# wzx99/DCFP

Measured on AMD Instinct MI355X. Metric: training images/sec at 1024x2048 DeepLabv3-R101, higher is better.
Workload: dtype f32; 1 GPU; DeepLabv3-resnet101+ASPP os8, 4x3x1024x2048 per GPU, CE+0.4*deepsup CE (fused upsample), 3x3 stride-1 convs with >= 256 channels as fp32 Winograd F(2x2,3x3) (fwd / dgrad / wgrad), all other convs direct implicit GEMM, EIC step, SGD m0.9 wd5e-4; global_batch=4, parallelism=dp1

## Files before the change

dcfp_amd/_lib.py:

```python
import ctypes as C
import os
import subprocess
import threading

_HERE = os.path.dirname(os.path.abspath(__file__))
LIB_PATH = os.environ.get("DCFP_LIB") or os.path.join(_HERE, "libdcfp_hip.so")
CSRC = os.path.join(_HERE, "csrc")

_lib = None
_lock = threading.Lock()


class ConvDesc(C.Structure):
    _fields_ = [(n, C.c_int32) for n in
                ("N", "Cin", "H", "W", "Cout", "KH", "KW", "stride", "pad", "dil", "Hout", "Wout",
                 "x_pitch", "dy_pitch")]


class ConvF16Desc(C.Structure):
    _fields_ = [(n, C.c_int32) for n in
                ("N", "H", "W", "Cin8", "x_pitch", "Cout", "K", "stride", "pad", "dil", "Hout", "Wout",
                 "y_pitch", "y_off", "res_pitch", "res_off", "relu")]


# ... 54 lines not shown

AUG_SATURATION, AUG_HUE = 1, 2
SGD_CHUNK = 16384
CONV_FWD, CONV_DGRAD, CONV_WGRAD = 0, 1, 2
E_BADDESC, E_UNSUPPORTED, E_WORKSPACE = -1, -2, -3

_P, _I, _L, _F, _Z = C.c_void_p, C.c_int, C.c_int64, C.c_float, C.c_size_t
_D = C.POINTER(ConvDesc)
_R = C.POINTER(BnRunning)
_H = C.POINTER(ConvF16Desc)
_H8 = C.POINTER(ConvF8Desc)

SIGNATURES = {
    "dcfp_abi_version": (_I, []),
    "dcfp_conv2d_workspace_bytes": (_Z, [_D, _I]),
    "dcfp_conv2d_wp_layout": (_I, [_D, _I, C.POINTER(WpEntry)]),
    "dcfp_conv2d_permute_weights_multi_f32": (_I, [_P, _I, _L, _P]),
    "dcfp_conv2d_pitch_supported": (_I, [_D]),
    "dcfp_conv2d_kernel_name": (_I, [_D, _I, C.c_char_p, _I]),
    "dcfp_conv2d_executed_fraction": (C.c_double, [_D, _I]),
    "dcfp_conv2d_workspace_is_scratch": (_I, [_D, _I]),
    "dcfp_conv2d_dgrad_fanin_supported": (_I, [_D]),
    "dcfp_conv2d_dgrad_fanin_f32_nchw": (_I, [_D, _P, _L, _P, _P, _P, _P, _P, _Z, _I, _P]),
    "dcfp_conv2d_dgrad_fanin_red_slots": (_L, [_D]),
    "dcfp_conv2d_dgrad_fanin_red_f32_nchw": (_I, [_D, _P, _L, _P, _P, _P, _P, _P, _P, _P, _P, _P, _Z, _I, _P]),
    "dcfp_bn_bwd_sums_from_partials_f32": (_I, [_P, _L, _I, _P, _F, _P, _P, _P, _P, _P]),
    "dcfp_conv2d_xform_bytes": (_Z, [_D]),
    "dcfp_conv2d_fwd_keep_f32_nchw": (_I, [_D, _P, _P, _P, _L, _P, _Z, _P, _P, _Z, _P]),
    "dcfp_conv2d_wgrad_kept_f32_nchw": (_I, [_D, _P, _L, _P, _Z, _P, _P, _Z, _P]),
    "dcfp_conv2d_fwd_f32_nchw": (_I, [_D, _P, _P, _P, _P, _L, _P, _Z, _I, _P]),
    "dcfp_conv2d_fwd_fused_f32_nchw": (_I, [_D, _P, _P, _P, _P, _P, _I, _P, _P, _Z, _I, _P]),
    "dcfp_conv2d_dgrad_f32_nchw": (_I, [_D, _P, _L, _P, _P, _I, _P, _Z, _I, _P]),
    "dcfp_conv2d_wgrad_f32_nchw": (_I, [_D, _P, _L, _P, _P, _P, _P, _Z, _P]),
    "dcfp_bn_workspace_bytes": (_Z, [_I, _I, _I]),
    "dcfp_bn_stats_f32": (_I, [_P, _L, _I, _I, _I, _P, _P, _R, _P, _Z, _P]),
    "dcfp_bn_apply_f32": (_I, [_P, _P, _P, _P, _P, _F, _P, _I, _P, _L, _I, _I, _I, _I, _I, _P]),
    "dcfp_bn_bwd_reduce_f32": (_I, [_P, _L, _P, _P, _L, _P, _P, _P, _P, _F, _I, _I, _I, _I, _P, _P, _P, _P,
                                    _P, _Z, _P]),
    "dcfp_bn_update_running_f32": (_I, [_P, _P, _I, _F, _F, _P, _P, _P, _P]),
    "dcfp_syncbn_combine_f32": (_I, [_P, _I, _I, _P, _P, _P, _R, _P]),
    "dcfp_syncbn_p2p_mailbox_bytes": (_Z, [_I, _I]),
    "dcfp_p2p_alloc": (_I, [_Z, _I, C.POINTER(C.c_void_p)]),
    "dcfp_p2p_free": (_I, [_P]),
    "dcfp_p2p_export": (_I, [_P, _P]),
    "dcfp_p2p_import": (_I, [_P, C.POINTER(C.c_void_p)]),
    "dcfp_p2p_unmap": (_I, [_P]),
    "dcfp_syncbn_p2p_exchange_f32": (_I, [C.POINTER(C.c_void_p), _I, _I, C.c_uint32, _I, _P, _I, _I, _P, _R,
                                          C.c_uint32, _P, _P]),
    "dcfp_bn_apply_relu_mask_f32": (_I, [_P, _P, _P, _P, _P, _F, _P, _P, _P, _I, _I, _I, _P]),
    "dcfp_conv2d_fwd_stat_slots": (_L, [_D, _P, _L]),
    "dcfp_conv2d_fwd_stats_f32_nchw": (_I, [_D, _P, _P, _P, _L, _P, _P, _Z, _I, _P]),
    "dcfp_bn_stats_from_partials_f32": (_I, [_P, _L, _I, _I, _P, _P, _R, _P]),
    "dcfp_bn_bwd_apply_f32": (_I, [_P, _L, _P, _P, _L, _P, _P, _P, _P, _F, _P, _P, _F, _P, _I, _P, _P,
                                   _I, _I, _I, _I, _I, _P]),
    "dcfp_bn_bwd_fused_sync_bytes": (_Z, [_I, _I, _I]),
    "dcfp_bn_bwd_fused_f32": (_I, [_P, _L, _P, _P, _L, _P, _P, _P, _P, _F, _F, _I, _P, _P, _I, _I, _I, _I, _I,
                                   _P, _P, _P, _P, _P, _Z, C.c_uint32, C.c_uint32, _P, _P]),
    "dcfp_maxpool3x3s2_fwd_f32": (_I, [_P, _P, _P, _I, _I, _I, _I, _I, _I, _P]),
    "dcfp_maxpool3x3s2_bwd_f32": (_I, [_P, _P, _P, _I, _I, _I, _I, _I, _I, _P]),
    "dcfp_rowsum_f32": (_I, [_P, _L, _P, _F, _I, _I, _I, _P]),
    "dcfp_broadcast_hw_f32": (_I, [_P, _F, _P, _L, _I, _I, _I, _I, _P]),
    "dcfp_add_f32": (_I, [_P, _P, _P, _L, _P]),
    "dcfp_channel_scale_f32": (_I, [_P, _P, _P, _I, _I, _I, _P]),
    "dcfp_upsample_bilinear_fwd_f32": (_I, [_P, _P, _I, _I, _I, _I, _I, _I, _I, _P]),
    "dcfp_upsample_bilinear_bwd_f32": (_I, [_P, _P, _I, _I, _I, _I, _I, _I, _I, _P]),
    "dcfp_resize_bilinear_into_f32": (_I, [_P, _L, _I, _I, _I, _I, _P, _L, _I, _I, _I, _I, _P]),
# ... 94 lines not shown
```

dcfp_amd/csrc/conv_igemm2.hip:

```cpp
#include "igemm2_common.h"
#include <queue>
#include <vector>
#include <stdio.h>
#include <stdlib.h>

namespace {

__device__ __forceinline__ int wp_row(int m, int perm8) {
    if (!perm8) return m;
    const int j = m & 255;
    return (m & ~255) + 32 * (j & 7) + (j >> 3);
}

__global__ void __launch_bounds__(256)
permute_weights_kernel(const float* __restrict__ w, float* __restrict__ wp, int T, int Ck, int CkP,
                       int M, int Mpad, int sAm, int sAc, int perm8) {
    const long long total = (long long)T * CkP * Mpad;
    for (long long i = (long long)blockIdx.x * 256 + threadIdx.x; i < total;
         i += (long long)gridDim.x * 256) {
        const int m = wp_row((int)(i % Mpad), perm8);
        const long long r = i / Mpad;
        const int c = (int)(r % CkP);
        const int t = (int)(r / CkP);
        float v = 0.f;
        if (m < M && c < Ck) v = w[(long long)m * sAm + (long long)c * sAc + t];
        wp[i] = v;
    }
}

constexpr int kWpBlockElems = DCFP_WP_BLOCK_ELEMS;
__global__ void __launch_bounds__(256)
permute_weights_multi_kernel(const DcfpWpEntry* __restrict__ table, int n) {
    const long long blk = blockIdx.x;
    int lo = 0, hi = n - 1;
    while (lo < hi) {
        const int mid = (lo + hi + 1) >> 1;
        if (table[mid].first_block <= blk) lo = mid; else hi = mid - 1;
    }
    const DcfpWpEntry e = table[lo];
    const long long base = (blk - e.first_block) * kWpBlockElems;
    if (e.perm8 >= 2) {
        const long long pairs = (long long)e.CkP * e.Mpad;
#pragma unroll 1
        for (int u = 0; u < kWpBlockElems / 256; ++u) {
            const long long i = base + u * 256 + threadIdx.x;
            if (i >= pairs) return;
            wino_filter2_pair(e.w, e.sAm, e.sAc, e.perm8 == 3, e.M, e.Ck, e.Mpad, i, e.wp);
        }
        return;
    }
    const long long total = (long long)e.T * e.CkP * e.Mpad;
#pragma unroll
    for (int u = 0; u < kWpBlockElems / 256; ++u) {
        const long long i = base + u * 256 + threadIdx.x;
        if (i >= total) return;
        const int m = wp_row((int)(i % e.Mpad), e.perm8);
        const long long r = i / e.Mpad;
        const int c = (int)(r % e.CkP);
        const int t = (int)(r / e.CkP);
        float v = 0.f;
        if (m < e.M && c < e.Ck) v = e.w[(long long)m * e.sAm + (long long)c * e.sAc + t];
        e.wp[i] = v;
    }
}

__device__ __forceinline__ float half_xor(float v, int mask) {
    switch (mask) {
        case 1: return __builtin_bit_cast(float, __builtin_amdgcn_ds_swizzle(__builtin_bit_cast(int, v), (1 << 10) | 0x1f));
        case 2: return __builtin_bit_cast(float, __builtin_amdgcn_ds_swizzle(__builtin_bit_cast(int, v), (2 << 10) | 0x1f));
        case 4: return __builtin_bit_cast(float, __builtin_amdgcn_ds_swizzle(__builtin_bit_cast(int, v), (4 << 10) | 0x1f));
        case 8: return __builtin_bit_cast(float, __builtin_amdgcn_ds_swizzle(__builtin_bit_cast(int, v), (8 << 10) | 0x1f));
        default: return __builtin_bit_cast(float, __builtin_amdgcn_ds_swizzle(__builtin_bit_cast(int, v), (16 << 10) | 0x1f));
    }
}

template <int TAPS, int TM, int TN, int WM, int WN, bool SD, bool ACC, int KB = 16>
__global__ void __launch_bounds__(64 * WM * WN, (TM * TN <= 8 && WM * WN == 4 && !ACC) ? 2 : 1)
igemm2_kernel(const Igemm2Params p) {
    constexpr int BK = KB;
    constexpr int NPART = BK / 4;
    constexpr int BM = WM * TM * 32, BN = WN * TN * 32, NT = 64 * WM * WN;
    constexpr int AX = BM / 4;
    constexpr int AROWS = (NT / AX) < BK ? (NT / AX) : BK;
// ... 1047 lines not shown
```

dcfp_amd/csrc/conv_wgrad.hip:

```cpp
#include "common.h"
#include <stdio.h>
#include <stdlib.h>
#include <string.h>
#include <type_traits>

int dcfp_wgrad3_launch(const float* dy, long long dy_nstride, const float* x, long long x_nstride,
                       float* out, int N, int M, int Cin, int T, int H, int W, int Ho, int Wo, int pad,
                       int dil, int Kpix, int kchunk, int splits, int tiles_m, int tiles_n,
                       hipStream_t stream);

namespace {

typedef float f32x16 __attribute__((ext_vector_type(16)));

constexpr int BK = 16;
constexpr int BKP = 20;

struct WgradParams {
    const float* dy;
    const float* x;
    float* out;
    long long dy_nstride, x_nstride;
    int N, M, Cin, Nn;
    int H, W, Ho, Wo, P, stride, pad, dil;
// ... 890 lines not shown
    const Plan pl = make_plan(d);
    const char* args = pl.cfg == 0 ? "4,4,2,2" : pl.cfg == 1 ? "2,4,2,2" : pl.cfg == 3 ? "4,2,2,2" :
                       pl.cfg == 4 ? "4,1,2,2" : pl.cfg == 5 ? "2,3,2,2" : "2,2,1,1";
    if (wgrad3_ok(d, pl.cfg)) return snprintf(buf, buf_len, "wgrad3_kernel<%d>", d->KH * d->KW);
    if (pl.wide) return snprintf(buf, buf_len, "wgrad_dma_kernel<%d,false,true>", d->KH * d->KW);
    if (wgrad_dma_ok(d, pl.cfg))
        return snprintf(buf, buf_len, "wgrad_dma_kernel<%d,%s>", d->KH * d->KW,
                        (wgrad_dma_mixed(d) && !(d->x_pitch && d->x_pitch != d->W)) ? "true" : "false");
    return snprintf(buf, buf_len, "wgrad2_kernel<%d,%s>", d->KH * d->KW, args);
}

bool dcfp_wino_wgrad_ok(int N, int H, int W, int d, int M, int C);
size_t dcfp_wino_wgrad_workspace_bytes(int N, int H, int W, int d, int M, int C);
double dcfp_wino_exec_fraction(int N, int H, int W, int d, int M, int Ck);
int dcfp_wino_wgrad_run(const float* dy, long long dy_nstride, int dy_pitch, const float* x, long long x_nstride,
                        int x_pitch, float* dw, int N, int M, int C, int H, int W, int d, void* workspace,
                        size_t workspace_bytes, hipStream_t stream, const float* xform_in = nullptr);
extern "C" size_t dcfp_conv2d_xform_bytes(const DcfpConvDesc* d);

static double wino_wgrad_fused_rate() {
    static const double v = [] { const char* e = getenv("DCFP_WINO_WGRAD_RATE"); return (e ? atof(e) : 118.0) * 1e12; }();
    return v;
}
static bool wino_wgrad_fused_forced() {
    static const bool v = [] { const char* e = getenv("DCFP_WINO_WGRAD_FUSED"); return e && atoi(e) == 2; }();
    return v;
}

bool dcfp_wino_wgrad_fused_ok(int N, int H, int W, int d, int M, int C, long long x_nstride, int x_pitch,
                              long long dy_nstride, int dy_pitch);
size_t dcfp_wino_wgrad_fused_workspace_bytes(int N, int H, int W, int d, int M, int C);
int dcfp_wino_wgrad_fused_run(const float* dy, long long dy_nstride, int dy_pitch, const float* x, long long x_nstride,
                              int x_pitch, float* dw, int N, int M, int C, int H, int W, int d, void* workspace,
                              size_t workspace_bytes, hipStream_t stream);

static int wino_wgrad_kind(const DcfpConvDesc* d) {
    static const int mode = [] { const char* e = getenv("DCFP_CONV_WINOGRAD"); return e ? atoi(e) : 1; }();
    if (mode == 0) return 0;
    if (d->KH != 3 || d->KW != 3 || d->stride != 1 || d->pad != d->dil || d->Hout != d->H || d->Wout != d->W) return 0;
    if (math_bf16x3()) return 0;
    const int xp = d->x_pitch ? d->x_pitch : d->W, dyp = d->dy_pitch ? d->dy_pitch : d->Wout;
    const bool batched = dcfp_wino_wgrad_ok(d->N, d->H, d->W, d->dil, d->Cout, d->Cin);
    const bool fused = dcfp_wino_wgrad_fused_ok(d->N, d->H, d->W, d->dil, d->Cout, d->Cin, (long long)d->Cin * d->H * xp, xp,
                                                (long long)d->Cout * d->Hout * dyp, dyp);
    if (!batched && !fused) return 0;
    if (mode == 2) return fused ? 2 : 1;
    const double pix = (double)d->N * d->H * d->W;
    const double nominal = 2.0 * pix * d->Cout * (double)d->Cin * 9.0;
    const bool dense_d1 = wgrad_dma_mixed(d) && !(d->x_pitch && d->x_pitch != d->W);
    const bool ragged = d->Cout % 256 != 0 || (d->Cin * 9) % 256 != 0;
    const double dpad = ragged ? (double)((d->Cout + 31) / 32 * 32) / d->Cout * (double)((d->Cin * 9 + 255) / 256 * 256) / (d->Cin * 9) * 1.15
                               : 1.0;
    const double t_direct = nominal * dpad / (d->Cout < 128 ? 100e12 : dense_d1 ? 123e12 : 130e12);
    const double f = dcfp_wino_exec_fraction(d->N, d->H, d->W, d->dil, d->Cout, d->Cin);
    double t_b = 1e30, t_f = 1e30;
    if (batched) {
        const double tiles = f * 9.0 / 16.0 * pix;
        const double pad2 = (double)((d->Cout + 255) / 256 * 256) / d->Cout * (double)((d->Cin + 255) / 256 * 256) / d->Cin;
        t_b = nominal * f * pad2 / 125e12 + (4.0 * pix * d->Cin + 64.0 * tiles * d->Cin) / 4.2e12 +
              (4.0 * pix * d->Cout + 64.0 * tiles * d->Cout) / 5.0e12 + 30e-6;
    }
    if (fused) {
        const double pad64 = (double)((d->Cout + 63) / 64 * 64) / d->Cout * (double)((d->Cin + 63) / 64 * 64) / d->Cin;
        t_f = nominal * f * pad64 / wino_wgrad_fused_rate() + 40e-6;
    }
    if (fused && (t_f <= t_b || wino_wgrad_fused_forced())) return t_f < 0.97 * t_direct ? 2 : 0;
    return t_b < 0.97 * t_direct ? 1 : 0;
}
static bool wino_wgrad_pass(const DcfpConvDesc* d) { return wino_wgrad_kind(d) != 0; }

bool dcfp_wgrad_is_winograd(const DcfpConvDesc* d) { return wino_wgrad_pass(d); }
bool dcfp_wgrad_wants_xform(const DcfpConvDesc* d) { return wino_wgrad_kind(d) == 1; }

double dcfp_wgrad_exec_fraction(const DcfpConvDesc* d) {
    return wino_wgrad_pass(d) ? dcfp_wino_exec_fraction(d->N, d->H, d->W, d->dil, d->Cout, d->Cin) : 1.0;
}

size_t dcfp_conv2d_fwd_dgrad_workspace_bytes_(const DcfpConvDesc* d, int pass);

extern "C" size_t dcfp_conv2d_workspace_bytes(const DcfpConvDesc* d, int pass) {
    if (pass == DCFP_CONV_FWD || pass == DCFP_CONV_DGRAD) return dcfp_conv2d_fwd_dgrad_workspace_bytes_(d, pass);
    if (pass != DCFP_CONV_WGRAD || check_desc(d) != DCFP_OK) return 0;
    if (dcfp_stem_shape(d)) return dcfp_stem_wgrad_workspace_bytes(d);
    if (const int wk = wino_wgrad_kind(d)) {
        const size_t b1 = dcfp_wino_wgrad_ok(d->N, d->H, d->W, d->dil, d->Cout, d->Cin)
                              ? dcfp_wino_wgrad_workspace_bytes(d->N, d->H, d->W, d->dil, d->Cout, d->Cin) : 0;
        if (wk == 1) return b1;
        const size_t b2 = dcfp_wino_wgrad_fused_workspace_bytes(d->N, d->H, d->W, d->dil, d->Cout, d->Cin);
        const Plan pl = make_plan(d);
        const size_t b0 = pl.splits > 1 ? (size_t)pl.splits * d->Cout * d->Cin * d->KH * d->KW * sizeof(float) : 0;
        const size_t m = b1 > b0 ? b1 : b0;
        return b2 > m ? b2 : m;
    }
    const Plan pl = make_plan(d);
    if (pl.splits <= 1) return 0;
    return (size_t)pl.splits * d->Cout * d->Cin * d->KH * d->KW * sizeof(float);
}

extern "C" int dcfp_conv2d_wgrad_f32_nchw(const DcfpConvDesc* d, const float* dy,
                                          int64_t dy_nstride, const float* x, float* dw, float* db,
                                          void* workspace, size_t workspace_bytes,
                                          dcfp_stream_t stream) {
    int rc = check_desc(d);
    if (rc) return rc;
    if (!dy || !x || !dw) return DCFP_E_BADDESC;
    if (dcfp_gemv_shape(d) && !db)
        return dcfp_gemv_wgrad(d, dy, dy_nstride, x, dw, dcfp_s(stream));
    if (dcfp_stem_shape(d) && !db)
        return dcfp_stem_wgrad(d, dy, dy_nstride, x, dw, workspace, workspace_bytes, dcfp_s(stream));
    int wk = wino_wgrad_kind(d);
    if (wk == 2) {
        const int dyp = d->dy_pitch ? d->dy_pitch : d->Wout, xp = d->x_pitch ? d->x_pitch : d->W;
        const long long dyn = dy_nstride ? dy_nstride : (long long)d->Cout * d->Hout * dyp;
        if (!dcfp_wino_wgrad_fused_ok(d->N, d->H, d->W, d->dil, d->Cout, d->Cin, (long long)d->Cin * d->H * xp, xp, dyn, dyp))
            wk = dcfp_wino_wgrad_ok(d->N, d->H, d->W, d->dil, d->Cout, d->Cin) ? 1 : 0;
    }
    if (wk) {
        const int dyp = d->dy_pitch ? d->dy_pitch : d->Wout, xp = d->x_pitch ? d->x_pitch : d->W;
        const long long dyn = dy_nstride ? dy_nstride : (long long)d->Cout * d->Hout * dyp;
        if (db && dyp != d->Wout) return DCFP_E_UNSUPPORTED;
        if (wk == 2) {
            rc = dcfp_wino_wgrad_fused_run(dy, dyn, dyp, x, (long long)d->Cin * d->H * xp, xp, dw, d->N, d->Cout, d->Cin, d->H,
                                           d->W, d->dil, workspace, workspace_bytes, dcfp_s(stream));
        } else
            rc = dcfp_wino_wgrad_run(dy, dyn, dyp, x, (long long)d->Cin * d->H * xp, xp, dw, d->N, d->Cout, d->Cin, d->H, d->W,
                                     d->dil, workspace, workspace_bytes, dcfp_s(stream));
        if (rc) return rc;
        if (db)
            hipLaunchKernelGGL(bias_grad_kernel, dim3((unsigned)d->Cout), dim3(1024), 0, dcfp_s(stream), dy, dyn, db, d->N,
                               d->Hout * d->Wout, (int)((d->Hout * d->Wout) % 4 == 0 && dyn % 4 == 0 && dcfp_aligned16(dy)));
        DCFP_RETURN_LAUNCH();
    }
    const Plan pl = make_plan(d);
    const int T = d->KH * d->KW;
    const long long wn = (long long)d->Cout * d->Cin * T;
    const size_t need = pl.splits > 1 ? (size_t)pl.splits * wn * sizeof(float) : 0;
    if (need && (!workspace || workspace_bytes < need)) return DCFP_E_WORKSPACE;
    WgradParams p;
    p.dy = dy; p.x = x;
    p.out = pl.splits > 1 ? static_cast<float*>(workspace) : dw;
    p.x_pitch = d->x_pitch ? d->x_pitch : d->W;
    p.dy_pitch = d->dy_pitch ? d->dy_pitch : d->Wout;
    const bool pitched = p.x_pitch != d->W || p.dy_pitch != d->Wout;
    if (pitched && !dcfp_wgrad_pitch_ok(d)) return DCFP_E_UNSUPPORTED;
    if (db && p.dy_pitch != d->Wout) return DCFP_E_UNSUPPORTED;
    p.dy_nstride = dy_nstride ? dy_nstride : (long long)d->Cout * d->Hout * p.dy_pitch;
    p.x_nstride = (long long)d->Cin * d->H * p.x_pitch;
    p.N = d->N; p.M = d->Cout; p.Cin = d->Cin; p.Nn = d->Cin * T;
    p.H = d->H; p.W = d->W; p.Ho = d->Hout; p.Wo = d->Wout; p.P = d->Hout * d->Wout;
    p.stride = d->stride; p.pad = d->pad; p.dil = d->dil;
    if ((long long)d->N * p.P >= (1LL << 30)) return DCFP_E_UNSUPPORTED;
    p.Kpix = d->N * p.P;
    p.kchunk = pl.kchunk; p.splits = pl.splits; p.tiles_m = pl.tiles_m; p.tiles_n = pl.tiles_n;
    p.quad_ok = (d->Wout % 4 == 0) ? 1 : 0;
    p.batch = 1; p.dy_bstride = p.x_bstride = 0;
    {
// ... 8 lines not shown
    else if (pl.wide) {
        const long long blocks = (long long)pl.tiles_m * pl.tiles_n * pl.splits;
        if (blocks > 0x7fffffffLL) return DCFP_E_UNSUPPORTED;
        rc = T == 1 ? launch_dma<1, false, true>(p, blocks, dcfp_s(stream)) : launch_dma<9, false, true>(p, blocks, dcfp_s(stream));
    } else if (wgrad_dma_ok(d, pl.cfg)) {
        const long long blocks = (long long)pl.tiles_m * pl.tiles_n * pl.splits;
        if (blocks > 0x7fffffffLL) return DCFP_E_UNSUPPORTED;
        rc = T == 1 ? (pl.half ? launch_dma<1, false, false, false, true>(p, blocks, dcfp_s(stream)) : launch_dma<1, false>(p, blocks, dcfp_s(stream)))
                    : (wgrad_dma_mixed(d) && p.x_pitch == d->W) ? launch_dma<9, true>(p, blocks, dcfp_s(stream))
                                                                 : launch_dma<9, false>(p, blocks, dcfp_s(stream));
    } else
        rc = T == 1 ? launch_taps<1>(p, pl, dcfp_s(stream)) : launch_taps<9>(p, pl, dcfp_s(stream));
    if (rc) return rc;
    if (pl.splits > 1) {
        if (wn % 4 == 0 && dcfp_aligned16(workspace) && dcfp_aligned16(dw)) {
            const long long n4 = wn / 4;
            hipLaunchKernelGGL(splitk_reduce_vec4_kernel, dim3((unsigned)((n4 + 255) / 256)), dim3(256), 0,
                               dcfp_s(stream), static_cast<const float*>(workspace), dw, n4, wn, pl.splits);
        } else {
            long long b = (wn + 255) / 256;
            if (b > 4096) b = 4096;
            hipLaunchKernelGGL(splitk_reduce_kernel, dim3((unsigned)b), dim3(256), 0, dcfp_s(stream),
                               static_cast<const float*>(workspace), dw, wn, pl.splits);
        }
    }
    if (db) {
        hipLaunchKernelGGL(bias_grad_kernel, dim3((unsigned)d->Cout), dim3(1024), 0, dcfp_s(stream),
                           dy, p.dy_nstride, db, d->N, p.P,
                           (int)(p.P % 4 == 0 && p.dy_nstride % 4 == 0 && dcfp_aligned16(dy) && p.dy_pitch == d->Wout));
    }
    DCFP_RETURN_LAUNCH();
}

extern "C" int dcfp_conv2d_wgrad_kept_f32_nchw(const DcfpConvDesc* d, const float* dy, int64_t dy_nstride,
                                               const float* xform, size_t xform_bytes, float* dw, void* workspace,
                                               size_t workspace_bytes, dcfp_stream_t stream) {
    int rc = check_desc(d);
    if (rc) return rc;
    if (!dy || !xform || !dw) return DCFP_E_BADDESC;
    const size_t need = dcfp_conv2d_xform_bytes(d);
    if (need == 0) return DCFP_E_UNSUPPORTED;
    if (xform_bytes < need || !dcfp_aligned16(xform)) return DCFP_E_WORKSPACE;
    const int dyp = d->dy_pitch ? d->dy_pitch : d->Wout;
    const long long dyn = dy_nstride ? dy_nstride : (long long)d->Cout * d->Hout * dyp;
    return dcfp_wino_wgrad_run(dy, dyn, dyp, nullptr, 0, 0, dw, d->N, d->Cout, d->Cin, d->H, d->W, d->dil, workspace,
                               workspace_bytes, dcfp_s(stream), xform);
}
```

dcfp_amd/csrc/conv_winograd3.hip:

```cpp
#include "wino_patch.h"
#include <stdlib.h>

namespace {

constexpr int GBK = 8;
constexpr int GKH = 144;
constexpr int GHALF = 2 * GKH;
constexpr int GCOMP = 2 * GHALF;
constexpr int GSTAGE = 16 * GCOMP;
constexpr unsigned kSat = 0xffffffffu;

struct WinoWgParams {
    const float* x_base;
    unsigned x_bytes;
    const float* dy_base;
    unsigned dy_bytes;
    const unsigned* table;
    unsigned table_bytes;
    float* out;
    int M, C, mblocks, cblocks, nblk;
    unsigned x_chan_bytes, dy_chan_bytes;
    int kchunk;
    long long T16;
    int d;
// ... 361 lines not shown
    splits = (pl.T16 + kchunk - 1) / kchunk;
    pl.splits = (int)splits;
    pl.kchunk = (int)kchunk;
    pl.table_floats = (pl.T16 / 2 * 8 + 63) / 64 * 64;
    pl.slab_floats = (long long)pl.splits * 16 * M * C;
    return pl;
}

}

bool dcfp_wino_wgrad_fused_enabled() {
    static const int v = [] { const char* e = getenv("DCFP_WINO_WGRAD_FUSED"); return e ? atoi(e) : 1; }();
    return v != 0;
}

bool dcfp_wino_wgrad_fused_ok(int N, int H, int W, int d, int M, int C, long long x_nstride, int x_pitch,
                              long long dy_nstride, int dy_pitch) {
    if (!dcfp_wino_wgrad_fused_enabled()) return false;
    if (M < 48 || C < 48) return false;
    if (x_pitch <= 0) x_pitch = W;
    if (dy_pitch <= 0) dy_pitch = W;
    if (wg_mode(N, H, W, d, M, C, x_nstride, x_pitch, dy_nstride, dy_pitch) < 0) return false;
    const WgPlan pl = wg_plan(N, H, W, d, M, C);
    if (pl.T16 >= (1LL << 30) || pl.T16 / 2 * 32 >= 0x7fffff00LL) return false;
    if (16LL * M * C * 4 >= 0x7fffff00LL) return false;
    return (long long)pl.mblocks * pl.cblocks * pl.splits < (1LL << 28);
}

size_t dcfp_wino_wgrad_fused_workspace_bytes(int N, int H, int W, int d, int M, int C) {
    const WgPlan pl = wg_plan(N, H, W, d, M, C);
    return (size_t)(pl.table_floats + pl.slab_floats) * sizeof(float);
}

int dcfp_wino_wgrad_fused_run(const float* dy, long long dy_nstride, int dy_pitch, const float* x, long long x_nstride,
                              int x_pitch, float* dw, int N, int M, int C, int H, int W, int d, void* workspace,
                              size_t workspace_bytes, hipStream_t stream) {
    if (x_pitch <= 0) x_pitch = W;
    if (dy_pitch <= 0) dy_pitch = W;
    const int mode = wg_mode(N, H, W, d, M, C, x_nstride, x_pitch, dy_nstride, dy_pitch);
    if (mode < 0) return DCFP_E_UNSUPPORTED;
    const WgPlan pl = wg_plan(N, H, W, d, M, C);
    if (!workspace || !dcfp_aligned16(workspace) || workspace_bytes < dcfp_wino_wgrad_fused_workspace_bytes(N, H, W, d, M, C))
        return DCFP_E_WORKSPACE;
    unsigned* table = static_cast<unsigned*>(workspace);
    float* slabs = static_cast<float*>(workspace) + pl.table_floats;
    const int lead = mode == 4 ? 0 : 4;
    const long long npairs = pl.T16 / 2;
    hipLaunchKernelGGL(wino_wg_table_kernel, dim3((unsigned)((npairs + 255) / 256)), dim3(256), 0, stream, table, npairs, pl.T,
                       N, H, W, d, pl.TH, pl.TW, x_nstride, x_pitch, lead, dy_nstride, dy_pitch, mode);
    WinoWgParams p;
    p.x_base = x - lead;
    p.x_bytes = (unsigned)(((long long)(N - 1) * x_nstride + (long long)C * H * x_pitch + lead) * 4);
    p.dy_base = dy;
    p.dy_bytes = (unsigned)(((long long)(N - 1) * dy_nstride + (long long)M * H * dy_pitch) * 4);
    p.table = table;
    p.table_bytes = (unsigned)(npairs * 32);
    p.out = slabs;
    p.M = M; p.C = C; p.mblocks = pl.mblocks; p.cblocks = pl.cblocks;
    p.nblk = pl.mblocks * pl.cblocks * pl.splits;
    p.x_chan_bytes = (unsigned)((long long)H * x_pitch * 4);
    p.dy_chan_bytes = (unsigned)((long long)H * dy_pitch * 4);
    p.kchunk = pl.kchunk;
    p.T16 = pl.T16;
    p.d = d;
    const unsigned grid = (unsigned)(((p.nblk + 7) / 8) * 8);
    const size_t lds = (size_t)4 * GSTAGE * sizeof(float);
    auto launch = [&](auto kern) -> int {
        hipError_t e = hipFuncSetAttribute(reinterpret_cast<const void*>(kern), hipFuncAttributeMaxDynamicSharedMemorySize,
                                           (int)lds);
        if (e != hipSuccess) return (int)e;
        hipLaunchKernelGGL(kern, dim3(grid), dim3(256), lds, stream, p);
        hipError_t e2 = hipGetLastError();
        return e2 == hipSuccess ? DCFP_OK : (int)e2;
    };
    const bool ragged = (M % 64) != 0 || (C % 64) != 0;
    int rc;
#define DCFP_WG(DM_) (ragged ? launch(wino_wgrad_fused_kernel<DM_, true>) : launch(wino_wgrad_fused_kernel<DM_, false>))
    switch (mode) {
        case 1: rc = DCFP_WG(1); break;
        case 2: rc = DCFP_WG(2); break;
        default: rc = DCFP_WG(4); break;
    }
// ... 7 lines not shown
```

dcfp_amd/ops.py:

```python
import ctypes as C
import os
import weakref

import torch
import torch.distributed as dist

from . import _lib, arena, syncbn_p2p
from ._lib import ConvDesc, BnRunning, check

_ws_cache = {}
WEIGHT_EPOCH = [0]

_PROFILE = None


def profile_start():
    global _PROFILE
    _PROFILE = []


def profile_stop():
    global _PROFILE
    recs, _PROFILE = _PROFILE, None
    torch.cuda.synchronize()
# ... 357 lines not shown
    return int(_lib.lib().dcfp_conv2d_dgrad_fanin_red_slots(C.byref(d)))


def conv2d_dgrad_fanin_red(dy, w, xshape, fan_src, fan_mask, red_x, red_mask, red_mean, slots):
    _require(dy, "dy"); _require(fan_src, "fan_src"); _require(red_x, "red_x")
    w = w if w.is_contiguous() else w.contiguous()
    d = _desc(xshape, w.shape, 1, 0, 1)
    dy, ns = _batch_strided(dy)
    if tuple(fan_src.shape) != tuple(xshape) or not fan_src.is_contiguous():
        raise RuntimeError("conv2d_dgrad_fanin_red: fan_src must be a contiguous tensor of the input shape")
    if tuple(red_x.shape) != tuple(xshape) or not red_x.is_contiguous() or red_mean.numel() != xshape[1]:
        raise RuntimeError("conv2d_dgrad_fanin_red: red_x / red_mean must match the input shape")
    dx = torch.empty(xshape, dtype=torch.float32, device=dy.device)
    part = torch.empty((slots, xshape[1], 2), dtype=torch.float32, device=dy.device)
    ws, valid = _conv_workspace(w, _lib.CONV_DGRAD, d)
    _timed("conv_dgrad_red", d, _conv_flops(d), lambda: check(
        _lib.lib().dcfp_conv2d_dgrad_fanin_red_f32_nchw(C.byref(d), _p(dy), ns, _p(w), _p(dx), _p(fan_src), _p(fan_mask),
                                                        _p(red_x), _p(red_mask), _p(red_mean), _p(part), _p(ws),
                                                        ws.numel(), valid, _stream()), "conv2d_dgrad_fanin_red"))
    return dx, part


def bn_bwd_sums_from_partials(part, var, eps, dgamma=None, dbeta=None):
    slots, Cc, _ = part.shape
    s = torch.empty((2, Cc), dtype=torch.float32, device=part.device)
    if dgamma is None:
        dgamma = torch.empty(Cc, dtype=torch.float32, device=part.device)
    _timed("bn_bwd_reduce", None, 8.0 * part.numel() / 2, lambda: check(
        _lib.lib().dcfp_bn_bwd_sums_from_partials_f32(_p(part), slots, Cc, _p(var), float(eps), _p(s[0]), _p(s[1]),
                                                      _p(dgamma), _p(dbeta), _stream()), "bn_bwd_sums_from_partials"))
    return s[0], s[1], dgamma


def conv2d_wgrad(dy, x, wshape, stride, pad, dil, need_bias=False, dw=None, db=None, xform=None):
    _require(dy, "dy"); _require(x, "x")
    xp, dp = _pitch_of(x), _pitch_of(dy)
    if not xp:
        x = x.contiguous()
    d = _desc(x.shape, wshape, stride, pad, dil, xp, dp)
    if dp:
        ns = dy.stride(0)
    else:
        dy, ns = _batch_strided(dy)
    L = _lib.lib()
    nbytes = L.dcfp_conv2d_workspace_bytes(C.byref(d), _lib.CONV_WGRAD)
    ws = _workspace("conv_scratch", nbytes, x.device)
    if dw is None:
        dw = torch.empty(wshape, dtype=torch.float32, device=x.device)
    elif tuple(dw.shape) != tuple(wshape) or not dw.is_contiguous():
        raise RuntimeError("conv2d_wgrad: dw must be a contiguous tensor of the weight shape")
    if need_bias and db is None:
        db = torch.empty((wshape[0],), dtype=torch.float32, device=x.device)
    if xform is not None and not need_bias and L.dcfp_conv2d_xform_bytes(C.byref(d)) == xform.numel():
        _timed("conv_wgrad", d, _conv_flops(d), lambda: check(
            L.dcfp_conv2d_wgrad_kept_f32_nchw(C.byref(d), _p(dy), ns, _p(xform), xform.numel(), _p(dw), _p(ws), ws.numel(),
                                              _stream()), "conv2d_wgrad_kept"))
        return dw, None
    _timed("conv_wgrad", d, _conv_flops(d), lambda: check(
        L.dcfp_conv2d_wgrad_f32_nchw(C.byref(d), _p(dy), ns, _p(x), _p(dw), _p(db) if need_bias else None, _p(ws),
                                     ws.numel(), _stream()), "conv2d_wgrad"))
    return dw, (db if need_bias else None)


def add_into(dst, src):
    check(_lib.lib().dcfp_add_f32(_p(dst), _p(src), _p(dst), dst.numel(), _stream()), "add")


def wgrad_into_param(dy, x, w, bias, stride, pad, dil, keep=None):
    tw, kw = arena.grad_target(w)
    tb, kb = arena.grad_target(bias) if bias is not None else (None, 0)
    xform = keep.pop("xform", None) if keep else None
    conv2d_wgrad(dy, x, tuple(w.shape), stride, pad, dil, need_bias=bias is not None, dw=tw, db=tb, xform=xform)
    dw = arena.grad_commit(w, tw, kw, add_into)
    db = arena.grad_commit(bias, tb, kb, add_into) if bias is not None else None
    return dw, db


class Conv2dFn(torch.autograd.Function):

    @staticmethod
    def forward(ctx, x, w, bias, stride, pad, dil):
        ctx.keep = {} if ctx.needs_input_grad[1] else None
        y = conv2d_fwd(x, w, bias, stride, pad, dil, keep=ctx.keep)
        ctx.save_for_backward(x)
        ctx.params = (w, bias)
        ctx.cfg = (stride, pad, dil)
        return y

    @staticmethod
    def backward(ctx, dy):
# ... 1456 lines not shown
```

include/dcfp_hip.h:

```cpp
#ifndef DCFP_HIP_H
#define DCFP_HIP_H

#include <stddef.h>
#include <stdint.h>

#ifdef __cplusplus
extern "C" {
#endif

#define DCFP_OK 0
#define DCFP_E_BADDESC (-1)
#define DCFP_E_UNSUPPORTED (-2)
#define DCFP_E_WORKSPACE (-3)

typedef void* dcfp_stream_t;

int dcfp_abi_version(void);

typedef struct DcfpConvDesc {
    int32_t N, Cin, H, W;
    int32_t Cout, KH, KW;
    int32_t stride, pad, dil;
    int32_t Hout, Wout;
    int32_t x_pitch, dy_pitch;
// ... 32 lines not shown
int dcfp_conv2d_dgrad_fanin_supported(const DcfpConvDesc* d);
int dcfp_conv2d_dgrad_fanin_f32_nchw(const DcfpConvDesc* d, const float* dy, int64_t dy_nstride, const float* w, float* dx,
                                     const float* fan_src, const void* fan_mask, void* workspace, size_t workspace_bytes,
                                     int wp_valid, dcfp_stream_t stream);
int64_t dcfp_conv2d_dgrad_fanin_red_slots(const DcfpConvDesc* d);
int dcfp_conv2d_dgrad_fanin_red_f32_nchw(const DcfpConvDesc* d, const float* dy, int64_t dy_nstride, const float* w,
                                         float* dx, const float* fan_src, const void* fan_mask, const float* red_x,
                                         const void* red_mask, const float* red_mean, float* red_part, void* workspace,
                                         size_t workspace_bytes, int wp_valid, dcfp_stream_t stream);
int dcfp_bn_bwd_sums_from_partials_f32(const float* partials, int64_t slots, int C, const float* var, float eps,
                                       float* sum_dy, float* sum_dy_xmu, float* dgamma ,
                                       float* dbeta , dcfp_stream_t stream);

int dcfp_conv2d_kernel_name(const DcfpConvDesc* d, int pass, char* buf, int buf_len);

double dcfp_conv2d_executed_fraction(const DcfpConvDesc* d, int pass);

int dcfp_conv2d_fwd_f32_nchw(const DcfpConvDesc* d, const float* x, const float* w,
                             const float* bias, float* y, int64_t y_nstride,
                             void* workspace, size_t workspace_bytes, int wp_valid,
                             dcfp_stream_t stream);
int dcfp_conv2d_fwd_fused_f32_nchw(const DcfpConvDesc* d, const float* x, const float* w,
                                   const float* scale, const float* shift, const float* residual,
                                   int relu, float* y, void* workspace, size_t workspace_bytes,
                                   int wp_valid, dcfp_stream_t stream);
int dcfp_conv2d_dgrad_f32_nchw(const DcfpConvDesc* d, const float* dy, int64_t dy_nstride,
                               const float* w, float* dx, int accumulate,
                               void* workspace, size_t workspace_bytes, int wp_valid,
                               dcfp_stream_t stream);
int dcfp_conv2d_wgrad_f32_nchw(const DcfpConvDesc* d, const float* dy, int64_t dy_nstride,
                               const float* x, float* dw, float* db,
                               void* workspace, size_t workspace_bytes,
                               dcfp_stream_t stream);

typedef struct DcfpBnRunning {
    float* running_mean;
    float* running_var;
    int64_t* num_batches_tracked;
    float momentum;
    int32_t pad_;
} DcfpBnRunning;
size_t dcfp_bn_workspace_bytes(int N, int C, int HW);
int dcfp_bn_stats_f32(const float* x, int64_t x_nstride, int N, int C, int HW,
                      float* mean, float* var, const DcfpBnRunning* run,
                      void* workspace, size_t workspace_bytes, dcfp_stream_t stream);
int dcfp_bn_apply_f32(const float* x, const float* mean, const float* var,
                      const float* gamma, const float* beta, float eps,
                      const float* residual, int relu, float* y, int64_t y_nstride,
                      int N, int C, int HW, int W, int y_pitch, dcfp_stream_t stream);
int dcfp_bn_bwd_reduce_f32(const float* dy, int64_t dy_nstride, const float* x,
                           const float* y, int64_t y_nstride, const float* mean,
                           const float* var, const float* gamma, const float* beta, float eps,
                           int relu, int N, int C, int HW,
                           float* sum_dy, float* sum_dy_xmu, float* dgamma ,
                           float* dbeta ,
                           void* workspace, size_t workspace_bytes, dcfp_stream_t stream);
int64_t dcfp_conv2d_fwd_stat_slots(const DcfpConvDesc* d, const float* y, int64_t y_nstride);
int dcfp_conv2d_fwd_stats_f32_nchw(const DcfpConvDesc* d, const float* x, const float* w, float* y,
                                   int64_t y_nstride, float* stat_partials, void* workspace,
                                   size_t workspace_bytes, int wp_valid, dcfp_stream_t stream);
int dcfp_bn_stats_from_partials_f32(const float* partials, int64_t slots, int slot_count, int C,
                                    float* mean, float* var, const DcfpBnRunning* run , dcfp_stream_t stream);
int dcfp_syncbn_combine_f32(const float* gathered, int world, int C, float* mean, float* var,
                            float* total_count, const DcfpBnRunning* run , dcfp_stream_t stream);
#define DCFP_P2P_HANDLE_BYTES 64
size_t dcfp_syncbn_p2p_mailbox_bytes(int world, int cap_floats);
// ... 278 lines not shown
```

Baseline: 12.28 images/s.

## Tile weight permutation through LDS and cache Winograd wgrad index tables

The weight-permutation kernel now stages 16x32 (or 8x64 for Winograd) tiles of filters in shared memory. This gives coalesced reads and writes for the plain permute and for the Winograd filter transform, which now writes vectorized float4 outputs. Separately, the fused Winograd wgrad tile-index table, which depends only on shapes and strides, is built once per shape/stream key and cached in Python, so the table-build kernel no longer launches on every wgrad call. The cost is more shared memory per permute block and a cache keyed on pointer-free layout parameters that persists for the process.

```diff
diff --git a/dcfp_amd/_lib.py b/dcfp_amd/_lib.py
--- a/dcfp_amd/_lib.py
+++ b/dcfp_amd/_lib.py
@@ -110,6 +110,9 @@
     "dcfp_conv2d_fwd_fused_f32_nchw": (_I, [_D, _P, _P, _P, _P, _P, _I, _P, _P, _Z, _I, _P]),
     "dcfp_conv2d_dgrad_f32_nchw": (_I, [_D, _P, _L, _P, _P, _I, _P, _Z, _I, _P]),
     "dcfp_conv2d_wgrad_f32_nchw": (_I, [_D, _P, _L, _P, _P, _P, _P, _Z, _P]),
+    "dcfp_conv2d_wgrad_table_bytes": (_Z, [_D, _L]),
+    "dcfp_conv2d_wgrad_table_build": (_I, [_D, _L, _P, _Z, _P]),
+    "dcfp_conv2d_wgrad_tab_f32_nchw": (_I, [_D, _P, _L, _P, _P, _P, _P, _Z, _P, _Z, _P]),
     "dcfp_bn_workspace_bytes": (_Z, [_I, _I, _I]),
     "dcfp_bn_stats_f32": (_I, [_P, _L, _I, _I, _I, _P, _P, _R, _P, _Z, _P]),
     "dcfp_bn_apply_f32": (_I, [_P, _P, _P, _P, _P, _F, _P, _I, _P, _L, _I, _I, _I, _I, _I, _P]),
diff --git a/dcfp_amd/csrc/conv_igemm2.hip b/dcfp_amd/csrc/conv_igemm2.hip
--- a/dcfp_amd/csrc/conv_igemm2.hip
+++ b/dcfp_amd/csrc/conv_igemm2.hip
@@ -29,8 +29,105 @@
 }
 
 constexpr int kWpBlockElems = DCFP_WP_BLOCK_ELEMS;
+constexpr int kWpTilePairs = 512;
+constexpr int kWpLdsFloats = 16 * (32 + 1) * 9;
+
+template <int TAPS, int NC, int NM>
+__device__ __forceinline__ void wp_stage_tile(const DcfpWpEntry& e, int c0, int p0, int perm8, float* lds) {
+    constexpr int ROW = (NM + 1) * TAPS;
+    const bool m_fast = e.sAm < e.sAc;
+#pragma unroll 2
+    for (int i = threadIdx.x; i < NC * NM * TAPS; i += 256) {
+        int cl, ml, t;
+        if (m_fast) {
+            cl = i / (NM * TAPS);
+            const int r = i - cl * (NM * TAPS);
+            ml = r / TAPS; t = r - ml * TAPS;
+        } else {
+            ml = i / (NC * TAPS);
+            const int r = i - ml * (NC * TAPS);
+            cl = r / TAPS; t = r - cl * TAPS;
+        }
+        const int c = c0 + cl, m = wp_row(p0 + ml, perm8);
+        float v = 0.f;
+        if (m < e.M && c < e.Ck) v = e.w[(long long)m * e.sAm + (long long)c * e.sAc + t];
+        lds[cl * ROW + ml * TAPS + t] = v;
+    }
+}
+
+template <int TAPS>
+__device__ __forceinline__ void wp_copy_tiles(const DcfpWpEntry& e, long long blk, float* lds) {
+    constexpr int NC = 16, NM = 32, ROW = (NM + 1) * TAPS;
+    constexpr int PER_BLOCK = kWpTilePairs * TAPS >= kWpBlockElems ? 1 : kWpBlockElems / (kWpTilePairs * TAPS);
+    const int ncb = e.CkP / NC, npb = e.Mpad / NM;
+    const long long tiles = (long long)ncb * npb;
+    const bool m_fast = e.sAm < e.sAc;
+#pragma unroll 1
+    for (int k = 0; k < PER_BLOCK; ++k) {
+        const long long u = blk * PER_BLOCK + k;
+        if (u >= tiles) return;
+        const int cb = m_fast ? (int)(u / npb) : (int)(u % ncb), pb = m_fast ? (int)(u % npb) : (int)(u / ncb);
+        if (k) __syncthreads();
+        wp_stage_tile<TAPS, NC, NM>(e, cb * NC, pb * NM, e.perm8, lds);
+        __syncthreads();
+        float* dst = e.wp + (long long)cb * NC * e.Mpad + pb * NM;
+#pragma unroll 2
+        for (int i = threadIdx.x; i < NC * NM * TAPS; i += 256) {
+            const int pl = i & (NM - 1), cl = (i / NM) & (NC - 1), t = i / (NC * NM);
+            dst[((long long)t * e.CkP + cl) * e.Mpad + pl] = lds[cl * ROW + pl * TAPS + t];
+        }
+    }
+}
+
+__device__ __forceinline__ void wp_wino_tiles(const DcfpWpEntry& e, long long blk, float* lds) {
+    constexpr int NC = 8, NM = 64, ROW = (NM + 1) * 9;
+    const int mblocks = e.Mpad / NM;
+    const long long tiles = (long long)(e.CkP / NC) * mblocks;
+    const bool flip = e.perm8 == 3;
+    const int q = threadIdx.x & 127, h = threadIdx.x >> 7;
+    const int ml = (q >> 6) * 32 + (q & 31), c1 = (q >> 5) & 1;
+#pragma unroll 1
+    for (int k = 0; k < kWpBlockElems / kWpTilePairs; ++k) {
+        const long long u = blk * (kWpBlockElems / kWpTilePairs) + k;
+        if (u >= tiles) return;
+        if (k) __syncthreads();
+        wp_stage_tile<9, NC, NM>(e, (int)(u / mblocks) * NC, (int)(u % mblocks) * NM, 0, lds);
+        __syncthreads();
+        float o[8][4];
+#pragma unroll
+        for (int kk = 0; kk < 4; ++kk) {
+            const float* src = lds + (2 * kk + c1) * ROW + ml * 9;
+            float g[9];
+#pragma unroll
+            for (int t = 0; t < 9; ++t) g[t] = src[flip ? 8 - t : t];
+            float r[4][3];
+#pragma unroll
+            for (int j = 0; j < 3; ++j) {
+                const float g0 = g[j], g1 = g[3 + j], g2 = g[6 + j];
+                r[0][j] = g0;
+                r[1][j] = 0.5f * ((g0 + g2) + g1);
+                r[2][j] = 0.5f * ((g0 + g2) - g1);
+                r[3][j] = g2;
+            }
+#pragma unroll
+            for (int ii = 0; ii < 2; ++ii) {
+                const float a = h ? r[2 + ii][0] : r[ii][0], b = h ? r[2 + ii][1] : r[ii][1],
+                            cc = h ? r[2 + ii][2] : r[ii][2];
+                o[4 * ii + 0][kk] = a;
+                o[4 * ii + 1][kk] = 0.5f * ((a + cc) + b);
+                o[4 * ii + 2][kk] = 0.5f * ((a + cc) - b);
+                o[4 * ii + 3][kk] = cc;
+            }
+        }
+        f32x4* dst = reinterpret_cast<f32x4*>(e.wp) + (u * 16 + 8 * h) * 128 + q;
+#pragma unroll
+        for (int x = 0; x < 8; ++x) dst[x * 128] = f32x4{o[x][0], o[x][1], o[x][2], o[x][3]};
+    }
+}
+
 __global__ void __launch_bounds__(256)
 permute_weights_multi_kernel(const DcfpWpEntry* __restrict__ table, int n) {
+    __shared__ float lds[kWpLdsFloats];
     const long long blk = blockIdx.x;
     int lo = 0, hi = n - 1;
     while (lo < hi) {
@@ -38,17 +135,16 @@
         if (table[mid].first_block <= blk) lo = mid; else hi = mid - 1;
     }
     const DcfpWpEntry e = table[lo];
+    if (e.perm8 >= 2) {
+        wp_wino_tiles(e, blk - e.first_block, lds);
+        return;
+    }
+    if ((e.T == 1 || e.T == 9) && e.CkP % 16 == 0 && e.Mpad % 32 == 0) {
+        if (e.T == 9) wp_copy_tiles<9>(e, blk - e.first_block, lds);
+        else wp_copy_tiles<1>(e, blk - e.first_block, lds);
+        return;
+    }
     const long long base = (blk - e.first_block) * kWpBlockElems;
-    if (e.perm8 >= 2) {
-        const long long pairs = (long long)e.CkP * e.Mpad;
-#pragma unroll 1
-        for (int u = 0; u < kWpBlockElems / 256; ++u) {
-            const long long i = base + u * 256 + threadIdx.x;
-            if (i >= pairs) return;
-            wino_filter2_pair(e.w, e.sAm, e.sAc, e.perm8 == 3, e.M, e.Ck, e.Mpad, i, e.wp);
-        }
-        return;
-    }
     const long long total = (long long)e.T * e.CkP * e.Mpad;
 #pragma unroll
     for (int u = 0; u < kWpBlockElems / 256; ++u) {
diff --git a/dcfp_amd/csrc/conv_wgrad.hip b/dcfp_amd/csrc/conv_wgrad.hip
--- a/dcfp_amd/csrc/conv_wgrad.hip
+++ b/dcfp_amd/csrc/conv_wgrad.hip
@@ -946,7 +946,10 @@
 size_t dcfp_wino_wgrad_fused_workspace_bytes(int N, int H, int W, int d, int M, int C);
 int dcfp_wino_wgrad_fused_run(const float* dy, long long dy_nstride, int dy_pitch, const float* x, long long x_nstride,
                               int x_pitch, float* dw, int N, int M, int C, int H, int W, int d, void* workspace,
-                              size_t workspace_bytes, hipStream_t stream);
+                              size_t workspace_bytes, hipStream_t stream, const void* kept_table, size_t kept_table_bytes);
+size_t dcfp_wino_wgrad_fused_table_bytes(int N, int H, int W, int d);
+int dcfp_wino_wgrad_fused_table_build(int N, int M, int C, int H, int W, int d, long long x_nstride, int x_pitch,
+                                      long long dy_nstride, int dy_pitch, void* table, size_t table_bytes, hipStream_t stream);
 
 static int wino_wgrad_kind(const DcfpConvDesc* d) {
     static const int mode = [] { const char* e = getenv("DCFP_CONV_WINOGRAD"); return e ? atoi(e) : 1; }();
@@ -1011,13 +1014,38 @@
     return (size_t)pl.splits * d->Cout * d->Cin * d->KH * d->KW * sizeof(float);
 }
 
-extern "C" int dcfp_conv2d_wgrad_f32_nchw(const DcfpConvDesc* d, const float* dy,
-                                          int64_t dy_nstride, const float* x, float* dw, float* db,
-                                          void* workspace, size_t workspace_bytes,
-                                          dcfp_stream_t stream) {
+static bool wgrad_runs_fused_wino(const DcfpConvDesc* d, int64_t dy_nstride) {
+    if (wino_wgrad_kind(d) != 2) return false;
+    const int dyp = d->dy_pitch ? d->dy_pitch : d->Wout, xp = d->x_pitch ? d->x_pitch : d->W;
+    const long long dyn = dy_nstride ? dy_nstride : (long long)d->Cout * d->Hout * dyp;
+    return dcfp_wino_wgrad_fused_ok(d->N, d->H, d->W, d->dil, d->Cout, d->Cin, (long long)d->Cin * d->H * xp, xp, dyn, dyp);
+}
+
+extern "C" size_t dcfp_conv2d_wgrad_table_bytes(const DcfpConvDesc* d, int64_t dy_nstride) {
+    if (check_desc(d) != DCFP_OK || dy_nstride < 0) return 0;
+    if (!wgrad_runs_fused_wino(d, dy_nstride)) return 0;
+    return dcfp_wino_wgrad_fused_table_bytes(d->N, d->H, d->W, d->dil);
+}
+
+extern "C" int dcfp_conv2d_wgrad_table_build(const DcfpConvDesc* d, int64_t dy_nstride, void* table, size_t table_bytes,
+                                             dcfp_stream_t stream) {
+    int rc = check_desc(d);
+    if (rc) return rc;
+    if (dy_nstride < 0) return DCFP_E_BADDESC;
+    if (dcfp_conv2d_wgrad_table_bytes(d, dy_nstride) == 0) return DCFP_E_UNSUPPORTED;
+    const int dyp = d->dy_pitch ? d->dy_pitch : d->Wout, xp = d->x_pitch ? d->x_pitch : d->W;
+    const long long dyn = dy_nstride ? dy_nstride : (long long)d->Cout * d->Hout * dyp;
+    return dcfp_wino_wgrad_fused_table_build(d->N, d->Cout, d->Cin, d->H, d->W, d->dil, (long long)d->Cin * d->H * xp, xp, dyn,
+                                             dyp, table, table_bytes, dcfp_s(stream));
+}
+
+static int wgrad_run(const DcfpConvDesc* d, const float* dy, int64_t dy_nstride, const float* x, float* dw, float* db,
+                     const void* kept_table, size_t kept_table_bytes, void* workspace, size_t workspace_bytes,
+                     dcfp_stream_t stream) {
     int rc = check_desc(d);
     if (rc) return rc;
     if (!dy || !x || !dw) return DCFP_E_BADDESC;
+    if (kept_table && !wgrad_runs_fused_wino(d, dy_nstride)) return DCFP_E_UNSUPPORTED;
     if (dcfp_gemv_shape(d) && !db)
         return dcfp_gemv_wgrad(d, dy, dy_nstride, x, dw, dcfp_s(stream));
     if (dcfp_stem_shape(d) && !db)
@@ -1035,7 +1063,7 @@
         if (db && dyp != d->Wout) return DCFP_E_UNSUPPORTED;
         if (wk == 2) {
             rc = dcfp_wino_wgrad_fused_run(dy, dyn, dyp, x, (long long)d->Cin * d->H * xp, xp, dw, d->N, d->Cout, d->Cin, d->H,
-                                           d->W, d->dil, workspace, workspace_bytes, dcfp_s(stream));
+                                           d->W, d->dil, workspace, workspace_bytes, dcfp_s(stream), kept_table, kept_table_bytes);
         } else
             rc = dcfp_wino_wgrad_run(dy, dyn, dyp, x, (long long)d->Cin * d->H * xp, xp, dw, d->N, d->Cout, d->Cin, d->H, d->W,
                                      d->dil, workspace, workspace_bytes, dcfp_s(stream));
@@ -1110,6 +1138,20 @@
     DCFP_RETURN_LAUNCH();
 }
 
+extern "C" int dcfp_conv2d_wgrad_f32_nchw(const DcfpConvDesc* d, const float* dy,
+                                          int64_t dy_nstride, const float* x, float* dw, float* db,
+                                          void* workspace, size_t workspace_bytes,
+                                          dcfp_stream_t stream) {
+    return wgrad_run(d, dy, dy_nstride, x, dw, db, nullptr, 0, workspace, workspace_bytes, stream);
+}
+
+extern "C" int dcfp_conv2d_wgrad_tab_f32_nchw(const DcfpConvDesc* d, const float* dy, int64_t dy_nstride, const float* x,
+                                              float* dw, float* db, const void* table, size_t table_bytes, void* workspace,
+                                              size_t workspace_bytes, dcfp_stream_t stream) {
+    if (!table) return DCFP_E_BADDESC;
+    return wgrad_run(d, dy, dy_nstride, x, dw, db, table, table_bytes, workspace, workspace_bytes, stream);
+}
+
 extern "C" int dcfp_conv2d_wgrad_kept_f32_nchw(const DcfpConvDesc* d, const float* dy, int64_t dy_nstride,
                                                const float* xform, size_t xform_bytes, float* dw, void* workspace,
                                                size_t workspace_bytes, dcfp_stream_t stream) {
diff --git a/dcfp_amd/csrc/conv_winograd3.hip b/dcfp_amd/csrc/conv_winograd3.hip
--- a/dcfp_amd/csrc/conv_winograd3.hip
+++ b/dcfp_amd/csrc/conv_winograd3.hip
@@ -417,9 +417,29 @@
     return (size_t)(pl.table_floats + pl.slab_floats) * sizeof(float);
 }
 
+size_t dcfp_wino_wgrad_fused_table_bytes(int N, int H, int W, int d) {
+    return (size_t)(wg_plan(N, H, W, d, 64, 64).T16 / 2) * 32;
+}
+
+int dcfp_wino_wgrad_fused_table_build(int N, int M, int C, int H, int W, int d, long long x_nstride, int x_pitch,
+                                      long long dy_nstride, int dy_pitch, void* table, size_t table_bytes, hipStream_t stream) {
+    if (x_pitch <= 0) x_pitch = W;
+    if (dy_pitch <= 0) dy_pitch = W;
+    const int mode = wg_mode(N, H, W, d, M, C, x_nstride, x_pitch, dy_nstride, dy_pitch);
+    if (mode < 0) return DCFP_E_UNSUPPORTED;
+    const WgPlan pl = wg_plan(N, H, W, d, M, C);
+    const long long npairs = pl.T16 / 2;
+    if (!table || !dcfp_aligned16(table) || table_bytes < (size_t)npairs * 32) return DCFP_E_WORKSPACE;
+    const int lead = mode == 4 ? 0 : 4;
+    hipLaunchKernelGGL(wino_wg_table_kernel, dim3((unsigned)((npairs + 255) / 256)), dim3(256), 0, stream,
+                       static_cast<unsigned*>(table), npairs, pl.T, N, H, W, d, pl.TH, pl.TW, x_nstride, x_pitch, lead,
+                       dy_nstride, dy_pitch, mode);
+    DCFP_RETURN_LAUNCH();
+}
+
 int dcfp_wino_wgrad_fused_run(const float* dy, long long dy_nstride, int dy_pitch, const float* x, long long x_nstride,
                               int x_pitch, float* dw, int N, int M, int C, int H, int W, int d, void* workspace,
-                              size_t workspace_bytes, hipStream_t stream) {
+                              size_t workspace_bytes, hipStream_t stream, const void* kept_table, size_t kept_table_bytes) {
     if (x_pitch <= 0) x_pitch = W;
     if (dy_pitch <= 0) dy_pitch = W;
     const int mode = wg_mode(N, H, W, d, M, C, x_nstride, x_pitch, dy_nstride, dy_pitch);
@@ -427,12 +447,16 @@
     const WgPlan pl = wg_plan(N, H, W, d, M, C);
     if (!workspace || !dcfp_aligned16(workspace) || workspace_bytes < dcfp_wino_wgrad_fused_workspace_bytes(N, H, W, d, M, C))
         return DCFP_E_WORKSPACE;
-    unsigned* table = static_cast<unsigned*>(workspace);
+    const long long npairs = pl.T16 / 2;
+    if (kept_table && (!dcfp_aligned16(kept_table) || kept_table_bytes < (size_t)npairs * 32)) return DCFP_E_WORKSPACE;
+    const unsigned* table = kept_table ? static_cast<const unsigned*>(kept_table) : static_cast<const unsigned*>(workspace);
     float* slabs = static_cast<float*>(workspace) + pl.table_floats;
+    if (!kept_table) {
+        const int rc = dcfp_wino_wgrad_fused_table_build(N, M, C, H, W, d, x_nstride, x_pitch, dy_nstride, dy_pitch, workspace,
+                                                         (size_t)npairs * 32, stream);
+        if (rc) return rc;
+    }
     const int lead = mode == 4 ? 0 : 4;
-    const long long npairs = pl.T16 / 2;
-    hipLaunchKernelGGL(wino_wg_table_kernel, dim3((unsigned)((npairs + 255) / 256)), dim3(256), 0, stream, table, npairs, pl.T,
-                       N, H, W, d, pl.TH, pl.TW, x_nstride, x_pitch, lead, dy_nstride, dy_pitch, mode);
     WinoWgParams p;
     p.x_base = x - lead;
     p.x_bytes = (unsigned)(((long long)(N - 1) * x_nstride + (long long)C * H * x_pitch + lead) * 4);
diff --git a/dcfp_amd/ops.py b/dcfp_amd/ops.py
--- a/dcfp_amd/ops.py
+++ b/dcfp_amd/ops.py
@@ -413,6 +413,25 @@
     return s[0], s[1], dgamma
 
 
+_WG_TABLES = {}
+
+
+def _wgrad_table(d, ns, device):
+    L = _lib.lib()
+    nbytes = L.dcfp_conv2d_wgrad_table_bytes(C.byref(d), ns)
+    if not nbytes:
+        return None
+    xp, dp = d.x_pitch or d.W, d.dy_pitch or d.Wout
+    key = (device.index, torch.cuda.current_stream().cuda_stream, d.N, d.H, d.W, d.dil, d.Cin * d.H * xp, xp,
+           ns or d.Cout * d.Hout * dp, dp)
+    tab = _WG_TABLES.get(key)
+    if tab is None or tab.numel() < nbytes:
+        tab = torch.empty(int(nbytes), dtype=torch.uint8, device=device)
+        check(L.dcfp_conv2d_wgrad_table_build(C.byref(d), ns, _p(tab), tab.numel(), _stream()), "conv2d_wgrad_table_build")
+        _WG_TABLES[key] = tab
+    return tab
+
+
 def conv2d_wgrad(dy, x, wshape, stride, pad, dil, need_bias=False, dw=None, db=None, xform=None):
     _require(dy, "dy"); _require(x, "x")
     xp, dp = _pitch_of(x), _pitch_of(dy)
@@ -437,6 +456,12 @@
             L.dcfp_conv2d_wgrad_kept_f32_nchw(C.byref(d), _p(dy), ns, _p(xform), xform.numel(), _p(dw), _p(ws), ws.numel(),
                                               _stream()), "conv2d_wgrad_kept"))
         return dw, None
+    tab = _wgrad_table(d, ns, x.device)
+    if tab is not None:
+        _timed("conv_wgrad", d, _conv_flops(d), lambda: check(
+            L.dcfp_conv2d_wgrad_tab_f32_nchw(C.byref(d), _p(dy), ns, _p(x), _p(dw), _p(db) if need_bias else None, _p(tab),
+                                             tab.numel(), _p(ws), ws.numel(), _stream()), "conv2d_wgrad_tab"))
+        return dw, (db if need_bias else None)
     _timed("conv_wgrad", d, _conv_flops(d), lambda: check(
         L.dcfp_conv2d_wgrad_f32_nchw(C.byref(d), _p(dy), ns, _p(x), _p(dw), _p(db) if need_bias else None, _p(ws),
                                      ws.numel(), _stream()), "conv2d_wgrad"))
diff --git a/include/dcfp_hip.h b/include/dcfp_hip.h
--- a/include/dcfp_hip.h
+++ b/include/dcfp_hip.h
@@ -88,6 +88,12 @@
                                const float* x, float* dw, float* db,
                                void* workspace, size_t workspace_bytes,
                                dcfp_stream_t stream);
+size_t dcfp_conv2d_wgrad_table_bytes(const DcfpConvDesc* d, int64_t dy_nstride);
+int dcfp_conv2d_wgrad_table_build(const DcfpConvDesc* d, int64_t dy_nstride, void* table, size_t table_bytes,
+                                  dcfp_stream_t stream);
+int dcfp_conv2d_wgrad_tab_f32_nchw(const DcfpConvDesc* d, const float* dy, int64_t dy_nstride,
+                                   const float* x, float* dw, float* db, const void* table, size_t table_bytes,
+                                   void* workspace, size_t workspace_bytes, dcfp_stream_t stream);
 
 typedef struct DcfpBnRunning {
     float* running_mean;
```

Result: no change. 12.30 images/s, median of 4 (+0.2%).
